# nyenyu12/BioInformatics-project-for-Shotgun-Metagenomics-Pseudo-alignment-shotgun-

Measured on AMD Instinct MI355X. Metric: reads/sec pseudo-aligned (k=31, 150bp) at 1/2/4/8 GPUs; % HBM roofline, higher is better.
Workload: dtype u8

## Files before the change

bioinformatics-project-for-shotgun-metagenomics-pseudo-alignment-shotgun-_amd/csrc/pa_align.hip:

```cpp
#include <hip/hip_runtime.h>

#include <algorithm>
#include <cstdio>
#include <cstdlib>
#include <cstring>
#include <type_traits>
#include <vector>

#include "pa_device.h"
#include "pa_internal.h"

using namespace pad;

namespace {

constexpr int kBlock = 256;
constexpr int kWaves = kBlock / 64;
constexpr uint32_t kSegMaxWaves = 16384;
constexpr uint32_t kSegSlackWaves = 8192, kSegSlackChunks = 5;
constexpr uint64_t kSegSlack = 64ull * kSegSlackChunks * kSegSlackWaves;
constexpr uint32_t kLdsGenomeCap = 2048;

enum : uint32_t { F_MRQ = 1, F_MKQ = 2, F_MG = 4 };

struct AlignArgs {
    const void *table;
    uint64_t cap;
    HomeCfg home;
    uint32_t G;
    int k;
    const uint32_t *class_genomes;
    const uint64_t *class_mask;
    const uint32_t *tile_cls;
    const uint64_t *tile_pk;
    uint64_t tile_n;
    const uint64_t *goff;
    const uint64_t *tile_lw;
    const uint64_t *tile_big;
    const void *tile_nb;
    uint64_t nb_base1, nb_split;
    const uint32_t *nbbig_ld;
    uint64_t nbbig_mask;
    int nb_spec;
    const uint32_t *tile_nbbig;
    const uint4 *tile_nbm;
    int mg_nb;
    const uint32_t *gblk;
    const uint64_t *bloom;
    const uint64_t *tile_rcp;
    const uint32_t *mm_bits;
    uint32_t mm_lg;
    const uint32_t *tile_rcnb;
    uint32_t bloom_lg;
    int walk_rounds;
    int tpos_local;
    uint32_t lane_maxpend;
    int lane_noanchor;
    int dbg_mode;
    const uint8_t *seq;
    const uint8_t *qual;
    const uint64_t *off;
    uint64_t n;
    uint64_t base;
    pa::DevParams prm;
    unsigned long long *stats;
    unsigned long long *uniq;
    unsigned long long *amb;
    unsigned long long *first;
    uint32_t *queue;
    unsigned long long *qcount;
// ... 676 lines not shown
                        uint32_t rank = 0;
                        for (uint32_t u = 0; u < nt; u++) {
                            const uint32_t h = ws.touched[u];
                            rank += h < g && ld_agent(&ws.g_tot[h]) == mx;
                        }
                        if (o + rank < end) x.lists[o + rank] = g;
                    }
                }
            }
            __syncthreads();
            exact_restore(ws, nt, n_touched, n_cls);
        }
        if (threadIdx.x == 0 && x.detail == 1) x.len_out[r] = nc;
        __syncthreads();
    }
}


size_t fast_lds_bytes(uint32_t G, int wpl, bool need_q) {
    size_t cnt = G <= kLdsGenomeCap ? (((size_t)((G + 1) & ~1u) * 16 + 15) / 16 * 16) : 0;
    size_t wl = wpl == 1 ? fast_wave_bytes<1>(need_q) : wpl == 2 ? fast_wave_bytes<2>(need_q) : fast_wave_bytes<4>(need_q);
    return cnt + kWaves * wl;
}

const char *env(const char *name) { return std::getenv(name); }
bool env_is(const char *name, char c) { const char *e = env(name); return e && e[0] == c; }
uint64_t env_u64(const char *name, uint64_t unset) { const char *e = env(name); return e ? std::strtoull(e, nullptr, 10) : unset; }
int env_int(const char *name, int unset) { const char *e = env(name); return e ? std::atoi(e) : unset; }
int env_01(const char *name) { const char *e = env(name); return e ? e[0] == '1' : -1; }

struct Switches {
    bool no_qelide = env("PA_NO_QELIDE");
    bool no_lane = env_is("PA_NO_LANE", '1');
    uint64_t lane_grid = env_u64("PA_LANE_GRID", ~0ull);
    uint32_t lane_maxpend = (uint32_t)env_int("PA_LANE_MAXPEND", 96);
    int lane_noanchor = env_01("PA_LANE_NOANCHOR");
    uint64_t na_min = env_u64("PA_NA_MIN", 32768);
    bool na_seg = !env_is("PA_NA_SEG", '0');
    bool na_rcwalk = !env_is("PA_NA_RCWALK", '0');
    bool na_rcnb = !env_is("PA_NA_RCNB", '0');
    bool mm_bits = !env_is("PA_MM_BITS", '0');
    bool no_nbbig = env("PA_NO_NBBIG");
    bool no_nbm = env("PA_NO_NBM");
    bool no_mgnb = env("PA_NO_MGNB");
    int walk_rounds = env_int("PA_WALK_ROUNDS", 1);
    int dbg_mode = env_int("PA_DBG_MODE", 0);
};

using pa::int_c;
using pa::with_int;
using pa::with_nw;

template <class F>
auto with_filters(uint32_t flags, F &&f) {
    const auto with_mg = [&](auto need_q, auto win_q) {
        return (flags & F_MG) ? f(need_q, win_q, std::true_type{}) : f(need_q, win_q, std::false_type{});
    };
    if (flags & F_MKQ) return with_mg(std::true_type{}, std::true_type{});
    if (flags & F_MRQ) return with_mg(std::true_type{}, std::false_type{});
    return with_mg(std::false_type{}, std::false_type{});
}

template <bool WIN_Q, class F>
auto with_shape(int nw, bool nm4, F &&f) {
    return with_int<3, 2, 1>(nw, [&](auto w) {
        if constexpr (!WIN_Q && w() == 1)
// ... 103 lines not shown
        PA_TRY(resident_grid(kern.rc, kBlock, 0, want, grid));
        PA_TRY(launch_timed(prof, PA_PROF_LANE_RC, kern.rc, grid, 0, st, b));
        b.queue_na = a.queue_na2;
        b.queue_na_count = a.queue_na2_count;
    }
    PA_TRY(resident_grid(kern.na, kBlock, 0, want, grid));
    return launch_timed(prof, PA_PROF_LANE_NA, kern.na, grid, 0, st, b);
}

pa_status launch_exact(pa_index *prof, int nw, const ExactArgs &x, unsigned grid, hipStream_t st) {
    KernelTimer kt(prof, st, PA_PROF_EXACT);
    with_nw(nw, [&](auto w) {
        hipLaunchKernelGGL(k_align_exact<w()>, dim3(grid), dim3(kBlock), 0, st, x);
    });
    PA_HIP(hipGetLastError());
    return PA_OK;
}

constexpr unsigned kExactGrid = 512;

AlignArgs make_args(const pa_index *idx, const pa_reads *r, const pa::DevParams &p, uint64_t base, const Switches &sw) {
    AlignArgs a{};
    a.table = idx->table;
    a.cap = idx->cap;
    a.home = idx->home;
    a.G = idx->n_genomes;
    a.k = (int)std::max<int64_t>(idx->k, 0);
    a.class_genomes = idx->class_genomes;
    a.class_mask = idx->class_mask;
    a.tile_cls = idx->tile_cls;
    a.tile_pk = idx->tile_pk;
    a.goff = idx->goff;
    a.tile_lw = idx->tile_cls ? idx->tile_lw : nullptr;
    a.tile_nb = idx->tile_cls ? idx->tile_nb : nullptr;
    a.nb_spec = idx->nb_spec;
    a.nb_split = idx->tile_nb1 ? idx->nb_split : ~0ull;
    a.nb_base1 = idx->tile_nb1 ? (uint64_t)(uintptr_t)idx->tile_nb1 - idx->nb_split * (idx->nb_spec ? 8 : 4) : 0;
    a.nbbig_ld = (const uint32_t *)(a.tile_nb ? a.tile_nb : (const void *)a.tile_lw);
    a.nbbig_mask = 0;
    a.gblk = idx->tile_gblk;
    a.bloom = idx->tile_cls ? idx->bloom : nullptr;
    a.bloom_lg = idx->bloom_lg;
    a.tile_rcp = idx->tile_cls && sw.na_rcwalk ? idx->tile_rcp : nullptr;
    a.mm_bits = idx->tile_cls && sw.mm_bits ? idx->mm_bits : nullptr;
    a.mm_lg = idx->mm_lg;
    a.tile_rcnb = idx->tile_cls && sw.na_rcnb ? idx->tile_rcnb : nullptr;
    a.tile_n = idx->tile_cls ? idx->tile_n : 0;
    a.walk_rounds = sw.walk_rounds;
    a.tpos_local = idx->tpos_local;
    a.lane_maxpend = sw.lane_maxpend;
    a.lane_noanchor = sw.lane_noanchor < 0 ? a.bloom != nullptr : sw.lane_noanchor;
    a.dbg_mode = sw.dbg_mode;
    a.seq = r->seq;
    a.qual = r->qual;
    a.off = r->off;
    a.n = r->n;
    a.base = base;
    a.prm = p;
    return a;
}

struct DetailOut { uint8_t *type; uint32_t *qf, *hr, *len; const uint64_t *list_off; uint32_t *lists; };

pa_status exact_args(pa_index *idx, const pa_reads *r, const AlignArgs &a, const DetailOut *out, ExactArgs &x,
                     unsigned &grid) {
    const uint32_t wcap = std::max<uint32_t>(1, r->max_len);
// ... 469 lines not shown
```

bioinformatics-project-for-shotgun-metagenomics-pseudo-alignment-shotgun-_amd/csrc/pa_index.hip:

```cpp
#include <hip/hip_runtime.h>

#include <algorithm>
#include <cmath>
#include <cstdlib>
#include <cstring>
#include <chrono>
#include <memory>
#include <cstdio>
#include <string>
#include <vector>

#include "pa_device.h"
#include "pa_internal.h"

using namespace pad;

namespace {

constexpr int kBlock = 256;
constexpr int kRun = 16;
#ifndef PA_BATCHED_INSERT
#define PA_BATCHED_INSERT 1
#endif
constexpr bool kBatchedInsert = PA_BATCHED_INSERT != 0;
// ... 1221 lines not shown
            if (maybe) maybe = table_find<1, true>(table, hc.cap, kk, home_of<1>(kk, key_hash(kk), hc), slot, cls, tpos);
        }
        const uint64_t b = __ballot(maybe);
        if (lane == 0) rcp[j] = b;
    }
}

__global__ void k_mm_build(const Slot<1> *__restrict__ table, uint64_t cap, uint32_t *bits, uint32_t lg, int k) {
    const uint64_t stride = (uint64_t)gridDim.x * blockDim.x;
    for (uint64_t i = (uint64_t)blockIdx.x * blockDim.x + threadIdx.x; i < cap; i += stride) {
        const uint64_t key = table[i].key[0];
        if (key == EMPTY) continue;
        const uint32_t h = mm_bit(k == 31 ? key_minimizer_c<31>(key) : key_minimizer(key, k), lg);
        atomicOr(&bits[h >> 5], 1u << (h & 31));
    }
}

__global__ __launch_bounds__(256) void k_tile_walk(const uint32_t *__restrict__ tile_cls, const uint64_t *__restrict__ pk,
                                                   uint64_t n, uint32_t G, uint64_t *__restrict__ lw, uint64_t n_blocks) {
    const uint32_t lane = threadIdx.x & 63;
    const uint64_t nw = (uint64_t)gridDim.x * (blockDim.x >> 6);
    for (uint64_t j = (uint64_t)blockIdx.x * (blockDim.x >> 6) + (threadIdx.x >> 6); j < n_blocks; j += nw) {
        const uint64_t t = 64 * j + lane;
        const uint32_t v = t < n ? tile_cls[t] : NONE;
        const bool ok = v != NONE, rep = ok && (v & PA_TILE_REP);
        const bool spec = ok && !rep && (v & ~PA_TILE_REP) < G;
        const uint64_t a = __ballot(ok && !rep), b = __ballot(rep || spec);
        if (lane < 4) {
            const uint64_t w = lane == 0 ? (64 * j < n ? pk[2 * j] : 0ull)
                             : lane == 1 ? (64 * j + 32 < n ? pk[2 * j + 1] : 0ull)
                             : lane == 2 ? a : b;
            lw[4 * j + lane] = w;
        }
    }
}

template <int NW>
__global__ void k_table_order(Slot<NW> *table, HomeCfg hc) {
    const uint64_t cap = hc.cap;
    uint64_t i = (uint64_t)blockIdx.x * blockDim.x + threadIdx.x;
    const uint64_t stride = (uint64_t)gridDim.x * blockDim.x;
    for (; i < cap; i += stride) {
        if (table[i].key[0] == EMPTY || table[i == 0 ? cap - 1 : i - 1].key[0] != EMPTY) continue;
        auto at = [&](uint64_t t) { return i + t >= cap ? i + t - cap : i + t; };
        auto rel = [&](const Slot<NW> &s) {
            Key<NW> kk;
#pragma unroll
            for (int j = 0; j < NW; j++) kk.w[j] = s.key[j];
            const uint64_t h = home_of<NW>(kk, key_hash(kk), hc);
            return h >= i ? h - i : h + cap - i;
        };
        for (uint64_t t = 1;; t++) {
            const Slot<NW> x = table[at(t)];
            if (x.key[0] == EMPTY) break;
            const uint64_t hx = rel(x);
            uint64_t q = t;
            for (; q > 0; q--) {
                const Slot<NW> y = table[at(q - 1)];
                if (rel(y) <= hx) break;
                table[at(q)] = y;
            }
            if (q != t) table[at(q)] = x;
        }
    }
}

// ... 462 lines not shown
    size_t free_b = 0, total_b = 0;
    if (!(no_nb && no_nb[0] == '1') && pa::dev_mem_info(&free_b, &total_b) == hipSuccess && bytes <= free_b / 4) {
        PA_HIP(pa::dev_malloc(&idx->tile_nb, bytes));
        PA_HIP(hipMemsetAsync(idx->tile_nb, 0, bytes, st));
        pa::Bufs b(st);
        uint64_t *bb = nullptr;
        uint32_t bb_lg = 6;
        if (idx->n_kmers > 0) {
            while (bb_lg < 33 && (1ull << bb_lg) * 4 < idx->n_kmers) bb_lg++;
            size_t fb = 0, tb = 0;
            if (pa::dev_mem_info(&fb, &tb) != hipSuccess) fb = 0;
            while (bb_lg > 6 && (1ull << bb_lg) * 8 > fb / 4) bb_lg--;
            if ((1ull << bb_lg) * 64 >= idx->n_kmers * 8 && b.get(&bb, (1ull << bb_lg) * 8) == hipSuccess) {
                PA_HIP(hipMemsetAsync(bb, 0, (1ull << bb_lg) * 8, st));
                hipLaunchKernelGGL(k_bloom_build2<3>, dim3(grid_for(idx->cap) > 65536 ? 65536 : grid_for(idx->cap)),
                                   dim3(kBlock), 0, st, (const Slot<3> *)idx->table, idx->cap, bb, bb_lg);
            } else {
                bb = nullptr;
            }
        }
        hipLaunchKernelGGL(k_nb_sum3, dim3(grid_for(n) > 65536 ? 65536 : grid_for(n)), dim3(kBlock), 0, st,
                           idx->tile_pk, idx->tile_cls, n, (int)idx->k, (const Slot<3> *)idx->table, idx->home,
                           (uint32_t *)idx->tile_nb, bb, bb_lg);
        PA_HIP(hipGetLastError());
        PA_HIP(b.free(bb));
        idx->nb_spec = 0;
        idx->device_bytes += bytes;
        phase_mark("nb: three-word summaries");
    }
    idx->nb_pending = 0;
    return PA_OK;
}

template <int NW>
pa_status build_tiles_nw(pa_index *idx, hipStream_t st) {
    const uint32_t G = idx->n_genomes;
    const int k = (int)idx->k;
    const int wpt = build_run();
    const uint64_t mask0 = (2 * k - 64 * (NW - 1)) >= 64 ? ~0ull : ((1ull << (2 * k - 64 * (NW - 1))) - 1);
    Slot<NW> *table = (Slot<NW> *)idx->table;
    if (idx->tile_n > 0) {
        size_t free_b = 0, total_b = 0;
        if (pa::dev_mem_info(&free_b, &total_b) != hipSuccess || idx->tile_n * 7 + (2ull << 30) > free_b) idx->tile_n = 0;
    }
    if (idx->tile_n > 0) {
        const uint64_t n = idx->tile_n, nwords = n / 32 + 32;
        PA_HIP(pa::dev_malloc(&idx->tile_cls, n * 4));
        PA_HIP(pa::dev_malloc(&idx->tile_pk, nwords * 8));
        PA_HIP(hipMemsetAsync(idx->tile_cls, 0xFF, n * 4, st));
        hipLaunchKernelGGL(k_tile_pack, dim3(grid_for(nwords) > 65536 ? 65536 : grid_for(nwords)), dim3(kBlock), 0, st,
                           idx->codes, n, idx->tile_pk, nwords);
        {
            std::vector<uint64_t> ts(G + 1, 0);
            for (uint32_t g = 0; g < G; g++) {
                const uint64_t len = idx->h_goff[g + 1] - idx->h_goff[g];
                ts[g + 1] = ts[g] + ((uint64_t)k > len ? 0 : (len - k + 1 + wpt - 1) / wpt);
            }
            pa::Bufs b(st);
            uint64_t *d_ts = nullptr;
            PA_HIP(b.get(&d_ts, (G + 1) * 8));
            PA_HIP(hipMemcpyAsync(d_ts, ts.data(), (G + 1) * 8, hipMemcpyHostToDevice, st));
            if (ts[G] > 0) {
                hipLaunchKernelGGL(k_tile_cls_all<NW>, dim3(grid_for(ts[G])), dim3(kBlock), 0, st, idx->codes, idx->goff,
                                   d_ts, G, k, mask0, table, idx->home, idx->tile_cls, idx->class_genomes,
                                   idx->tpos_local, wpt);
                PA_HIP(hipGetLastError());
// ... 71 lines not shown
                    idx->bloom_lg = lg;
                    idx->device_bytes += (1ull << lg) * 8;
                }
                phase_mark("Bloom");
            }
            {
                const char *nm = std::getenv("PA_NO_MM");
                const uint32_t lg = 25;
                if (NW == 1 && !(nm && nm[0] == '1') && idx->bloom && idx->n_kmers / 9 <= (1ull << lg) / 4 &&
                    pa::dev_malloc(&idx->mm_bits, (1ull << lg) / 8) == hipSuccess) {
                    PA_HIP(hipMemsetAsync(idx->mm_bits, 0, (1ull << lg) / 8, st));
                    hipLaunchKernelGGL(k_mm_build, dim3(grid_for(idx->cap) > 65536 ? 65536 : grid_for(idx->cap)),
                                       dim3(kBlock), 0, st, (const Slot<1> *)table, idx->cap, idx->mm_bits, lg, k);
                    idx->mm_lg = lg;
                    idx->device_bytes += (1ull << lg) / 8;
                } else {
                    idx->mm_bits = nullptr;
                }
                phase_mark("minimizer bitmap");
            }
            {
                const char *nr = std::getenv("PA_NO_RCP");
                const uint64_t n_blocks = n / 64 + 5;
                if (NW == 1 && !(nr && nr[0] == '1') && pa::dev_malloc(&idx->tile_rcp, n_blocks * 8) == hipSuccess) {
                    hipLaunchKernelGGL(k_tile_rcp, dim3((unsigned)std::min<uint64_t>((n_blocks + 3) / 4, 1u << 20)),
                                       dim3(256), 0, st, idx->tile_cls, idx->tile_pk, n, k, (const Slot<1> *)table,
                                       idx->home, idx->bloom, idx->bloom_lg, idx->tile_rcp, n_blocks);
                    idx->device_bytes += n_blocks * 8;
                } else {
                    idx->tile_rcp = nullptr;
                }
                phase_mark("reverse-complement plane");
            }
        }
        PA_HIP(hipGetLastError());
        PA_HIP(hipStreamSynchronize(st));
        idx->device_bytes += n * 4 + nwords * 8;
    }
    return PA_OK;
}

template <int NW>
pa_status lookup_nw(const pa_index *idx, const uint8_t *d_kmers, uint64_t n, int64_t *d_cls, uint32_t *d_size,
                    hipStream_t st) {
    const int k = (int)idx->k;
    const uint64_t mask0 = (2 * k - 64 * (NW - 1)) >= 64 ? ~0ull : ((1ull << (2 * k - 64 * (NW - 1))) - 1);
    hipLaunchKernelGGL(k_lookup<NW>, dim3(grid_for(n)), dim3(kBlock), 0, st, (const Slot<NW> *)idx->table, idx->home,
                       d_kmers, n, k, mask0, idx->n_genomes, idx->class_genomes, d_cls, d_size);
    PA_HIP(hipGetLastError());
    return PA_OK;
}

template <int NW>
void extsim_slots_nw(const pa_index *idx, const uint32_t *d_group, uint32_t n_groups, unsigned long long *total,
                     unsigned long long *uniq, unsigned long long *ccount, hipStream_t st) {
    int use_lds = n_groups <= 4096;
    size_t shm = use_lds ? (size_t)n_groups * 8 : 0;
    unsigned grid = grid_for(idx->cap) > 4096 ? 4096 : grid_for(idx->cap);
    hipLaunchKernelGGL(k_extsim_slots<NW>, dim3(grid), dim3(kBlock), shm, st, (const Slot<NW> *)idx->table, idx->cap,
                       idx->n_genomes, d_group, n_groups, total, uniq, ccount, use_lds);
}

}

namespace pa {

void index_release(pa_index *idx) {
    index_release_coverage(idx);
    pa::dev_free(idx->table);
    pa::dev_free(idx->class_off);
    pa::dev_free(idx->class_size);
    pa::dev_free(idx->class_genomes);
    pa::dev_free(idx->class_mask);
    pa::dev_free(idx->codes);
    pa::dev_free(idx->goff);
    pa::dev_free(idx->fwd_len);
    idx->fwd_len = nullptr;
    pa::dev_free(idx->tile_cls);
    pa::dev_free(idx->tile_pk);
    pa::dev_free(idx->tile_lw);
    idx->tile_lw = nullptr;
    pa::dev_free(idx->tile_big);
    idx->tile_big = nullptr;
    idx->tile_big_mg = -1;
    pa::dev_free(idx->tile_nb);
    idx->tile_nb = nullptr;
    pa::dev_free(idx->tile_nb1);
    idx->tile_nb1 = nullptr;
    idx->nb_split = ~0ull;
    pa::dev_free(idx->tile_rcnb);
    idx->tile_rcnb = nullptr;
    pa::dev_free(idx->tile_nbbig);
    idx->tile_nbbig = nullptr;
    idx->tile_nbbig_mg = -1;
    pa::dev_free(idx->tile_nbm);
    idx->tile_nbm = nullptr;
    idx->tile_nbm_mg = -1;
    pa::dev_free(idx->bloom);
    idx->bloom = nullptr;
    pa::dev_free(idx->tile_rcp);
    idx->tile_rcp = nullptr;
    pa::dev_free(idx->mm_bits);
    idx->mm_bits = nullptr;
    pa::dev_free(idx->tile_gblk);
    idx->tile_gblk = nullptr;
    idx->bloom_lg = 0;
    idx->tile_cls = nullptr;
    idx->tile_pk = nullptr;
    pa::dev_free(idx->ws.ptr);
    pa::dev_free(idx->queue);
    pa::dev_free(idx->queue_hard);
    pa::dev_free(idx->queue_na);
    pa::dev_free(idx->queue_na2);
    pa::dev_free(idx->queue_na_keys);
// ... 9 lines not shown
    pa::dev_free(idx->qmask);
    pa::dev_free(idx->qdrop);
    idx->qmask = nullptr;
    idx->qdrop = nullptr;
    idx->qmask_cap = 0;
    idx->queue_na = nullptr;
    idx->na_count = nullptr;
    pa::dev_free(idx->counters);
    for (auto e : idx->ev_start) hipEventDestroy(e);
    for (auto e : idx->ev_stop) hipEventDestroy(e);
    for (auto &e : idx->kev) {
        hipEventDestroy(e.start);
        hipEventDestroy(e.stop);
    }
    idx->kev.clear();
    idx->table = nullptr;
}

pa_status index_build_rcnb(pa_index *idx, hipStream_t st) {
    if (!idx->rcnb_pending) return PA_OK;
    std::unique_ptr<PhaseTimer> own;
    if (!t_phase) own.reset(new PhaseTimer(st));
    PhaseScope ps(t_phase ? t_phase : own.get());
    Bufs b(st);
    uint64_t *bb = nullptr;
    uint32_t bb_lg = 6;
    PA_TRY(make_nb_bloom(idx, st, b, &bb, &bb_lg));
    return build_rcnb(idx, st, bb, bb_lg);
}

pa_status index_note_reads(pa_index *idx, uint64_t n, hipStream_t st) {
    idx->reads_seen += n;
    if (!idx->nb_pending || !nb_repaid(idx->reads_seen, idx->tile_n, idx->nw)) return PA_OK;
    return build_nb(idx, st);
}

pa_status index_prepare(pa_index *idx, hipStream_t st, uint64_t reads_hint, bool complete) {
    if (!idx->tiles_pending) {
        if (complete && idx->nb_pending &&
            (reads_hint == ~0ull || nb_repaid(idx->reads_seen + reads_hint, idx->tile_n, idx->nw))) {
            std::unique_ptr<PhaseTimer> own;
            if (!t_phase) own.reset(new PhaseTimer(st));
            PhaseScope ps(t_phase ? t_phase : own.get());
            return build_nb(idx, st);
        }
        return PA_OK;
    }
    idx->tiles_pending = 0;
    std::unique_ptr<PhaseTimer> own;
    if (!t_phase) own.reset(new PhaseTimer(st));
    PhaseScope ps(t_phase ? t_phase : own.get());
    const uint64_t bases = idx->h_goff.empty() ? 0 : idx->h_goff.back();
    idx->nb_skip = reads_hint != ~0ull && !nb_repaid(reads_hint, bases, idx->nw);
    pa_status rc = idx->nw == 3   ? build_tiles_nw<3>(idx, st)
                   : idx->nw == 2 ? build_tiles_nw<2>(idx, st)
                                  : build_tiles_nw<1>(idx, st);
    idx->nb_skip = 0;
    if (rc != PA_OK) {
        pa::dev_free(idx->tile_cls); pa::dev_free(idx->tile_pk); pa::dev_free(idx->tile_lw); pa::dev_free(idx->tile_nb);
        pa::dev_free(idx->tile_nb1);
        idx->tile_nb1 = nullptr, idx->nb_split = ~0ull, idx->rcnb_pending = 0;
        pa::dev_free(idx->tile_gblk); pa::dev_free(idx->bloom); pa::dev_free(idx->tile_rcp); pa::dev_free(idx->tile_rcnb);
        pa::dev_free(idx->mm_bits);
        idx->mm_bits = nullptr;
        idx->tile_rcnb = nullptr;
        idx->tile_cls = nullptr, idx->tile_pk = nullptr, idx->tile_lw = nullptr, idx->tile_nb = nullptr;
        idx->tile_gblk = nullptr, idx->bloom = nullptr, idx->bloom_lg = 0, idx->tile_n = 0, idx->tile_rcp = nullptr;
    }
    return rc;
}

pa_status index_build(pa_index *idx, const char *genomes, const uint64_t *goff, uint32_t n, int64_t k,
                      hipStream_t st, bool defer_tiles, uint8_t *dev_codes) {
    PhaseTimer tm(st);
    PhaseScope ps(&tm);
    idx->k = k;
    idx->nw = k > 0 ? key_words(k) : 1;
    idx->n_genomes = n;
    const bool both = idx->both_strands != 0;
    const uint64_t text_off = goff[0], fwd_total = goff[n] - goff[0];
    std::vector<uint64_t> fwd_goff, region_goff;
    if (both) {
        idx->h_fwd_len.resize(n);
        for (uint32_t g = 0; g < n; g++) {
            const uint64_t len = goff[g + 1] - goff[g];
            idx->h_fwd_len[g] = dev_codes ? (len ? (len - 1) / 2 : 0) : len;
        }
        if (!dev_codes) {
            fwd_goff.assign(goff, goff + n + 1);
            for (auto &o : fwd_goff) o -= goff[0];
            region_goff.assign(n + 1, 0);
            for (uint32_t g = 0; g < n; g++) region_goff[g + 1] = region_goff[g] + strand_region(idx->h_fwd_len[g]);
            goff = region_goff.data();
        }
    }
    idx->h_goff.assign(goff, goff + n + 1);
    const uint64_t total = goff[n] - goff[0];
// ... 367 lines not shown
```

bioinformatics-project-for-shotgun-metagenomics-pseudo-alignment-shotgun-_amd/csrc/pa_internal.h:

```cpp
#pragma once

#include <hip/hip_runtime.h>
#include <stdint.h>

#include <map>
#include <memory>
#include <string>
#include <type_traits>
#include <vector>

#include "../../include/pa.h"
#include "pa_home.h"

namespace pa {

void set_error(const std::string &msg);

pa_status hip_failed(hipError_t e, const char *where);
#define PA_STR2(x) #x
#define PA_STR(x) PA_STR2(x)
#define PA_HIP(call)                                                                              \
    do {                                                                                          \
        hipError_t e_ = (call);                                                                   \
        if (e_ != hipSuccess) return ::pa::hip_failed(e_, __FILE__ ":" PA_STR(__LINE__) " (" #call ")"); \
// ... 114 lines not shown

struct pa_index {
    int device = 0;
    int64_t k = 0;
    int nw = 1;
    uint32_t n_genomes = 0;
    void *table = nullptr;
    uint64_t cap = 0;
    pad::HomeCfg home{};
    uint64_t n_kmers = 0;
    uint64_t n_multi = 0;
    uint64_t *class_off = nullptr;
    uint32_t *class_size = nullptr;
    uint32_t *class_genomes = nullptr;
    uint64_t class_entries = 0;
    uint64_t *class_mask = nullptr;
    uint8_t *codes = nullptr;
    uint64_t *goff = nullptr;
    std::vector<uint64_t> h_goff;
    uint64_t total_windows = 0;
    int tpos_local = 0;
    uint64_t distinct_estimate = 0;
    int released = 0;
    int force_large = 0;
    int compact_table = 0;
    int both_strands = 0;
    std::vector<uint64_t> h_fwd_len;
    uint64_t *fwd_len = nullptr;
    uint64_t tile_n = 0;
    int tiles_pending = 0;
    uint32_t *tile_cls = nullptr;
    uint64_t *tile_pk = nullptr;
    uint64_t *tile_lw = nullptr;
    uint64_t *tile_big = nullptr;
    int64_t tile_big_mg = -1;
    void *tile_nb = nullptr;
    int nb_spec = 0;
    void *tile_nb1 = nullptr;
    uint64_t nb_split = ~0ull;
    uint32_t *tile_rcnb = nullptr;
    int rcnb_pending = 0;
    int rcnb_checks = 0;
    uint32_t *tile_nbbig = nullptr;
    int64_t tile_nbbig_mg = -1;
    uint4 *tile_nbm = nullptr;
    int64_t tile_nbm_mg = -1;
    int nb_skip = 0;
    int nb_pending = 0;
    uint64_t reads_seen = 0;
    uint32_t *tile_gblk = nullptr;
    uint64_t *bloom = nullptr;
    uint32_t *mm_bits = nullptr;
    uint32_t mm_lg = 0;
    uint64_t *tile_rcp = nullptr;
    uint32_t bloom_lg = 0;
    uint64_t device_bytes = 0;
    uint32_t *cov_head = nullptr;
    uint32_t *cov_first = nullptr;
    uint64_t cov_pairs = 0;
    uint64_t cov_bytes = 0;
    int cov_ready = 0;
    uint64_t epoch = 0;
    pa::Workspace ws;
    uint32_t *queue = nullptr;
    uint32_t *queue_hard = nullptr;
    uint32_t *queue_na = nullptr;
// ... 222 lines not shown
```

bioinformatics-project-for-shotgun-metagenomics-pseudo-alignment-shotgun-_amd/csrc/pa_lane.h:

```cpp

constexpr uint64_t kPosMask = (1ull << 40) - 1;
template <int NM>
struct LaneShape {
    static constexpr int MAXW = 64 * NM;
    static constexpr int NWD = NM == 2 ? 6 : 9;
    static constexpr int MAXLEN = 32 * NWD - 16;
    static constexpr int NB = NM + 1;
};
constexpr int kLaneMaxW = LaneShape<2>::MAXW;
constexpr int kLaneMaxLen = LaneShape<2>::MAXLEN;
constexpr int kLaneWords = LaneShape<2>::NWD;
#ifndef PA_LANE_MAXMIS
#define PA_LANE_MAXMIS 40
#endif
constexpr uint32_t kLaneMaxMis = PA_LANE_MAXMIS;
#ifndef PA_LANE_PROBES
#define PA_LANE_PROBES 4
#endif
#ifndef PA_LANE_SEEDS
#define PA_LANE_SEEDS 5
#endif
#ifndef PA_SEED_SLOTS
#define PA_SEED_SLOTS 2
#endif
// ... 220 lines not shown
    uint64_t P[NM];
    uint64_t F[NM];
    uint32_t qf;
    uint32_t uoff;
};

__device__ __forceinline__ uint64_t row_bits(const uint64_t *row, uint32_t o) {
    const uint32_t q = o >> 6, r = o & 63;
    const uint64_t hi = row[q] << r;
    return r ? (hi | (row[q + 1] >> (64 - r))) : hi;
}

template <int NW>
__device__ __forceinline__ Key<NW> row_key(const uint64_t *row, uint32_t w, int k) {
    Key<NW> K;
    if constexpr (NW == 1) {
        K.w[0] = row_bits(row, 2 * w) >> (64 - 2 * k);
    } else {
        static_assert(NW == 2 || NW == 3, "lane-path keys: one to three words");
#pragma unroll
        for (int j = 1; j < NW; j++) K.w[j] = row_bits(row, 2 * w + 2 * k - 64 * (NW - j));
        const int hb = 2 * k - 64 * (NW - 1);
        K.w[0] = hb ? row_bits(row, 2 * w) >> (64 - hb) : 0ull;
    }
    return K;
}

__device__ __forceinline__ uint32_t in_read_mask(uint32_t p0, uint32_t shift, uint32_t len) {
    const uint32_t lo = shift > p0 ? shift - p0 : 0u, hi = shift + len > p0 ? shift + len - p0 : 0u;
    return (hi >= 4 ? 0xFFFFFFFFu : ((1u << (8 * hi)) - 1)) & (lo >= 4 ? 0u : (0xFFFFFFFFu << (8 * lo)));
}


template <bool PLANES, int NWD = kLaneWords, int NB = 3>
__device__ __forceinline__ void lane_blocks(const AlignArgs &a, uint64_t A, uint32_t len, uint64_t (&gw)[NWD + 1],
                                            uint64_t (&pa3)[NB], uint64_t (&pb3)[NB]) {
    const uint64_t *lb = a.tile_lw + 4 * (A >> 6);
    const uint32_t r0 = (uint32_t)(A & 63), o = r0 >> 5, last = r0 + len - 1;
#pragma unroll
    for (int i = 0; i <= NWD; i++) {
        const uint32_t w = o + (uint32_t)i;
        gw[i] = 32 * w <= last ? lb[4 * (w >> 1) + (w & 1)] : 0ull;
    }
    if (PLANES) {
#pragma unroll
        for (int i = 0; i < NB; i++) {
            const ulonglong2 p = *(const ulonglong2 *)(lb + 4 * i + 2);
            pa3[i] = p.x;
            pb3[i] = p.y;
        }
    }
}

template <int NWD = kLaneWords>
__device__ __forceinline__ uint32_t lane_count_mismatches(const uint64_t *row, uint32_t len, uint64_t A,
                                                          const uint64_t (&gw)[NWD + 1]) {
    const uint32_t gr = (uint32_t)(2 * A & 63);
    uint32_t n = 0;
    const uint32_t qlast = (len - 1) >> 5, rl = len - 32 * qlast;
    const uint64_t tail = rl >= 32 ? ~0ull : ~0ull << (64 - 2 * rl);
#pragma unroll
    for (int i = 0; i < NWD; i++) {
        if (32 * i >= (int)len) break;
        const uint64_t gwi = gr ? ((gw[i] << gr) | (gw[i + 1] >> (64 - gr))) : gw[i];
        uint64_t d = row[i] ^ gwi;
        if ((uint32_t)i == qlast) d &= tail;
        n += __popcll((d | (d >> 1)) & 0x5555555555555555ull);
    }
    return n;
}
// ... 183 lines not shown
    for (int i = 1; i < NSEED; i++)
        if (at == i) {
            S.anc = stp[i] | ((uint64_t)sw(i) << 40);
            S.acls = scls[i];
        }
    if (S.acls >= a.G) {
        const int64_t e0 = (int64_t)(S.anc & kPosMask) - (int64_t)(S.anc >> 40);
        int64_t e1 = INT64_MIN, e2 = INT64_MIN;
        uint64_t t1 = 0, t2 = 0;
        uint32_t w1 = 0, c1 = 0, w2 = 0, c2 = 0;
#pragma unroll
        for (int i = 0; i < NSEED; i++) {
            const int64_t Ai = (int64_t)stp[i] - sw(i);
            if (stp[i] == ~0ull || Ai == e0 || Ai == e1 || e2 != INT64_MIN) continue;
            if (e1 == INT64_MIN) {
                e1 = Ai;
                t1 = stp[i], w1 = sw(i), c1 = scls[i];
            } else {
                e2 = Ai;
                t2 = stp[i], w2 = sw(i), c2 = scls[i];
            }
        }
        if (e1 != INT64_MIN) {
#ifdef PA_STATS
            atomicAdd(&a.dbg[26], 1ull);
#endif
#ifndef PA_LANE_RANK_WORDS4
#define PA_LANE_RANK_WORDS4 5
#endif
            constexpr int NR = NM == 2 ? PA_LANE_RANK_WORDS : PA_LANE_RANK_WORDS4;
            const uint32_t rlen = len < 32u * NR ? len : 32u * NR;
            const bool f0 = lane_fits(a, len, e0), f1 = lane_fits(a, len, e1), f2 = e2 != INT64_MIN && lane_fits(a, len, e2);
            uint64_t g0[NR + 1], g1[NR + 1], g2[NR + 1], u3[3];
            lane_blocks<false, NR>(a, f0 ? (uint64_t)e0 : 0, rlen, g0, u3, u3);
            lane_blocks<false, NR>(a, f1 ? (uint64_t)e1 : 0, rlen, g1, u3, u3);
            lane_blocks<false, NR>(a, f2 ? (uint64_t)e2 : 0, rlen, g2, u3, u3);
            const uint32_t m0 = f0 ? lane_count_mismatches<NR>(row, rlen, (uint64_t)e0, g0) : ~0u;
            const uint32_t m1 = f1 ? lane_count_mismatches<NR>(row, rlen, (uint64_t)e1, g1) : ~0u;
            const uint32_t m2 = f2 ? lane_count_mismatches<NR>(row, rlen, (uint64_t)e2, g2) : ~0u;
            uint32_t bj = 0, best = m0;
            if (m1 < best) best = m1, bj = 1;
            if (m2 < best) best = m2, bj = 2;
            if (bj == 1) {
                S.anc = t1 | ((uint64_t)w1 << 40), S.acls = c1;
            } else if (bj == 2) {
                S.anc = t2 | ((uint64_t)w2 << 40), S.acls = c2;
            }
        }
    }
    S.kind = LANE_WALK;
}

template <int NM, bool NEED_Q, bool WIN_Q, bool SEEDS = true, int NW = 1>
__device__ __forceinline__ void lane_prep(const AlignArgs &a, uint64_t r, unsigned long long cd, uint64_t *row,
                                          LaneRead<NM> &S) {
    using SH = LaneShape<NM>;
    static_assert(NM == 2 || !WIN_Q, "the window-quality masks cover 128 windows");
    constexpr int NWD = SH::NWD;
    S.kind = LANE_HARD;
    S.hr = S.nspec = S.nincl = 0;
#pragma unroll
    for (int i = 0; i < NM; i++) S.F[i] = 0;
    S.qf = 0;
    S.uoff = 0;
    const int k = a.k;
    const uint32_t flags = a.prm.flags;
    const uint64_t o = a.off[r];
    const uint32_t len = (uint32_t)(a.off[r + 1] - o);
    const uint64_t o0 = o & ~15ull;
// ... 158 lines not shown
    for (int i = 1; i < NSEED; i++)
        if (at == i) {
            S.anc = stp[i] | ((uint64_t)sw(i) << 40);
            S.acls = scls[i];
        }
    if (S.acls >= a.G) {
        const int64_t e0 = (int64_t)(S.anc & kPosMask) - (int64_t)(S.anc >> 40);
        int64_t e1 = INT64_MIN, e2 = INT64_MIN;
        uint64_t t1 = 0, t2 = 0;
        uint32_t w1 = 0, c1 = 0, w2 = 0, c2 = 0;
#pragma unroll
        for (int i = 0; i < NSEED; i++) {
            const int64_t Ai = (int64_t)stp[i] - sw(i);
            if (stp[i] == ~0ull || Ai == e0 || Ai == e1 || e2 != INT64_MIN) continue;
            if (e1 == INT64_MIN) {
                e1 = Ai;
                t1 = stp[i], w1 = sw(i), c1 = scls[i];
            } else {
                e2 = Ai;
                t2 = stp[i], w2 = sw(i), c2 = scls[i];
            }
        }
        if (e1 != INT64_MIN) {
#ifdef PA_STATS
            atomicAdd(&a.dbg[26], 1ull);
#endif
#ifndef PA_LANE_RANK_WORDS4
#define PA_LANE_RANK_WORDS4 5
#endif
            constexpr int NR = NM == 2 ? PA_LANE_RANK_WORDS : PA_LANE_RANK_WORDS4;
            const uint32_t rlen = len < 32u * NR ? len : 32u * NR;
            const bool f0 = lane_fits(a, len, e0), f1 = lane_fits(a, len, e1), f2 = e2 != INT64_MIN && lane_fits(a, len, e2);
            uint64_t g0[NR + 1], g1[NR + 1], g2[NR + 1], u3[3];
            lane_blocks<false, NR>(a, f0 ? (uint64_t)e0 : 0, rlen, g0, u3, u3);
            lane_blocks<false, NR>(a, f1 ? (uint64_t)e1 : 0, rlen, g1, u3, u3);
            lane_blocks<false, NR>(a, f2 ? (uint64_t)e2 : 0, rlen, g2, u3, u3);
            const uint32_t m0 = f0 ? lane_count_mismatches<NR>(row, rlen, (uint64_t)e0, g0) : ~0u;
            const uint32_t m1 = f1 ? lane_count_mismatches<NR>(row, rlen, (uint64_t)e1, g1) : ~0u;
            const uint32_t m2 = f2 ? lane_count_mismatches<NR>(row, rlen, (uint64_t)e2, g2) : ~0u;
            uint32_t bj = 0, best = m0;
            if (m1 < best) best = m1, bj = 1;
            if (m2 < best) best = m2, bj = 2;
            if (bj == 1) {
                S.anc = t1 | ((uint64_t)w1 << 40), S.acls = c1;
            } else if (bj == 2) {
                S.anc = t2 | ((uint64_t)w2 << 40), S.acls = c2;
            }
        }
    }
    S.kind = LANE_WALK;
}

template <int NM>
__device__ __forceinline__ uint64_t lane_any(const uint64_t (&m)[NM]) {
    uint64_t x = 0;
#pragma unroll
    for (int i = 0; i < NM; i++) x |= m[i];
    return x;
}
template <int NM>
__device__ __forceinline__ uint32_t lane_popc(const uint64_t (&m)[NM]) {
    uint32_t x = 0;
#pragma unroll
    for (int i = 0; i < NM; i++) x += (uint32_t)__popcll(m[i]);
    return x;
}

template <int NM>
__device__ __forceinline__ void range_mask(int32_t lo, int32_t hi, uint64_t (&r)[NM]) {
#pragma unroll
    for (int i = 0; i < NM; i++) {
        const int32_t b = 64 * i, l = lo - b, h = hi - b;
        r[i] = (h < 0 || l > 63) ? 0ull
                                 : ((l <= 0 ? ~0ull : (~0ull << l)) & (h >= 63 ? ~0ull : ((2ull << h) - 1)));
    }
}

template <int NM>
__device__ __forceinline__ void or_at(uint64_t (&m)[NM], uint64_t v, int32_t sft) {
#pragma unroll
    for (int i = 0; i < NM; i++) {
        const int32_t s = sft - 64 * i;
        m[i] |= (s >= 64 || s <= -32) ? 0ull : (s >= 0 ? v << s : v >> (-s));
    }
}

template <int NM>
__device__ __forceinline__ void shifted_planes(const uint64_t (&p)[NM + 1], uint32_t fr, uint64_t (&out)[NM]) {
#pragma unroll
    for (int i = 0; i < NM; i++) out[i] = fr ? (p[i] >> fr) | (p[i + 1] << (64 - fr)) : p[i];
}

template <bool WIN_Q, bool MG, int NW = 1, int SURE = lane_sure(WIN_Q, MG, 2, NW)>
__device__ __forceinline__ void lane_walk_150(const AlignArgs &a, const uint64_t *row, LaneRead<2> &S) {
    const int k = a.k;
    uint32_t W = S.W, len = S.len;
    asm volatile("" : "+v"(W), "+v"(len));
    const uint64_t atp = S.anc & kPosMask;
    const int64_t A = (int64_t)atp - (int64_t)(S.anc >> 40);
    const bool in_tile = A >= 0 && (uint64_t)A + W <= a.tile_n;
    const uint64_t Ac = in_tile ? (uint64_t)A : 0;
    const uint32_t gr = (uint32_t)(2 * Ac & 63);
    uint64_t gw[kLaneWords + 1], pa3[3], pb3[3];
    lane_blocks<true>(a, Ac, len, gw, pa3, pb3);
    const uint32_t g = S.acls < a.G ? S.acls : genome_of(a.goff, a.gblk, atp);
    S.g = g;
    const uint64_t gs = a.goff[g], ge = a.goff[g + 1];
    if (!in_tile || A < (int64_t)gs || (uint64_t)A + W - 1 + k > ge) {
        S.kind = LANE_HARD;
        return (void)LANE_HARD_WHY(4);
    }
    const uint32_t fr = (uint32_t)(Ac & 63);
    const uint64_t PA0 = fr ? (pa3[0] >> fr) | (pa3[1] << (64 - fr)) : pa3[0];
    const uint64_t PA1 = fr ? (pa3[1] >> fr) | (pa3[2] << (64 - fr)) : pa3[1];
    const uint64_t PB0 = fr ? (pb3[0] >> fr) | (pb3[1] << (64 - fr)) : pb3[0];
    const uint64_t PB1 = fr ? (pb3[1] >> fr) | (pb3[2] << (64 - fr)) : pb3[1];
    const uint64_t IX0 = PA0 | PB0, IX1 = PA1 | PB1;
    uint64_t U0 = 0, U1 = 0, V0 = 0, V1 = 0, NP0 = 0, NP1 = 0, NS0 = 0, NS1 = 0, NG0 = 0, NG1 = 0;
    uint32_t nmis = 0;
    const bool has_nb = a.tile_nb != nullptr;
    uint64_t epk = 0;
    uint32_t cpk = 0;
    uint32_t nnb = 0;
    const uint32_t qlast = (len - 1) >> 5, rl = len - 32 * qlast;
    const uint64_t tail = rl >= 32 ? ~0ull : ~0ull << (64 - 2 * rl);
    auto mismatch = [&](uint32_t e, auto &&sub) -> bool {
        const int32_t lo = (int32_t)e - k + 1 < 0 ? 0 : (int32_t)e - k + 1;
        const int32_t hi = (int32_t)e < (int32_t)W - 1 ? (int32_t)e : (int32_t)W - 1;
        if (lo > hi) return true;
        const uint64_t r0 = lo < 64 ? ((~0ull << lo) & (hi >= 63 ? ~0ull : ((2ull << hi) - 1))) : 0ull;
        const uint64_t r1 =
            hi >= 64 ? ((lo <= 64 ? ~0ull : (~0ull << (lo - 64))) & (hi >= 127 ? ~0ull : ((2ull << (hi - 64)) - 1)))
                     : 0ull;
        if (!((r0 & IX0) | (r1 & IX1))) return true;
        if (++nmis > 8) {
            if (nmis > kLaneMaxMis) return false;
            V0 |= r0;
// ... 235 lines not shown
    }
    if ((uint32_t)(__popcll(P0) + __popcll(P1)) > a.lane_maxpend) {
        S.kind = LANE_HARD;
        return (void)LANE_HARD_WHY(8);
    }
}

#ifndef PA_LANE_HALVES
#define PA_LANE_HALVES 1
#endif
template <bool MG>
__device__ __forceinline__ void lane_walk_halves(const AlignArgs &a, const uint64_t *row, LaneRead<4> &S) {
    const int64_t A = (int64_t)(S.anc & kPosMask) - (int64_t)(S.anc >> 40);
    const uint32_t len = S.len, W = S.W;
    S.nspec = S.nincl = S.hr = S.uoff = 0;
    S.P[2] = S.P[3] = 0;
    uint32_t cs = 0, sw = 0;
#pragma unroll 1
    for (uint32_t h = 0; h < 2; h++) {
        LaneRead<2> H;
        H.kind = LANE_WALK;
        H.F[0] = H.F[1] = 0;
        if (h == 0) {
            H.len = W > 128 ? 127 + (uint32_t)a.k : len;
            H.W = W > 128 ? 128u : W;
            H.anc = S.anc;
            H.acls = S.acls;
        } else {
            H.len = len - 128;
            H.W = W - 128;
            H.anc = (uint64_t)(A + 128);
            H.acls = S.g;
        }
        lane_walk_150<false, MG, 1, lane_sure(false, MG, 4, 1) ? 2 : 0>(a, row + 4 * h, H);
        if (h == 0) S.g = H.g;
        S.kind = H.kind;
        S.nspec += H.nspec, S.nincl += H.nincl, S.hr += H.hr, S.uoff += H.uoff & 255u;
        if (H.kind == LANE_WALK && (H.uoff & 0xFF00u)) {
            if (!cs) sw = 128 * h + ((H.uoff >> 16) & 255u);
            cs += (H.uoff >> 8) & 255u;
        }
        if (h == 0) {
            S.P[0] = H.P[0], S.P[1] = H.P[1];
        } else {
            S.P[2] = H.P[0], S.P[3] = H.P[1];
        }
        if (S.kind != LANE_WALK || W <= 128) break;
    }
    if (S.kind == LANE_WALK && cs && S.nspec < cs + (uint32_t)(a.prm.m > 0 ? a.prm.m : 1)) {
#pragma unroll
        for (uint32_t q = 0; q < 4; q++) S.P[q] = (sw >> 6) == q ? 1ull << (sw & 63) : 0ull;
        S.uoff = kLaneSure;
    }
}

template <int NM, bool WIN_Q, bool MG>
__device__ __forceinline__ void lane_walk_long(const AlignArgs &a, const uint64_t *row, LaneRead<NM> &S) {
    using SH = LaneShape<NM>;
    constexpr int NWD = SH::NWD;
    const int k = a.k;
    const uint32_t W = S.W, len = S.len;
    const uint64_t atp = S.anc & kPosMask;
    const int64_t A = (int64_t)atp - (int64_t)(S.anc >> 40);
    const bool in_tile = A >= 0 && (uint64_t)A + W <= a.tile_n;
    const uint64_t Ac = in_tile ? (uint64_t)A : 0;
    const uint32_t gr = (uint32_t)(2 * Ac & 63);
    uint64_t gw[NWD + 1], pa3[NM + 1], pb3[NM + 1];
// ... 1353 lines not shown
```

Baseline: 4.553 billion.

## Add overlapping walk-block records so lane walks read contiguous 128-byte spans

Builds a new device array in which each 64-base tile block gets a 128-byte record holding the packed words and masks of that block and the next three blocks. The lane walk and verification paths index this record instead of gathering up to three separate 32-byte tile_lw entries, so each read's genome window comes from one contiguous span. The cost is a table four times the size of tile_lw, an extra build kernel, and a free-memory check that skips the table when memory is short. It is on by default and can be turned off with PA_LW_RECORDS=0.

Result: no change. 4.554 billion, median of 3 (+0.0%).

```diff
diff --git a/bioinformatics-project-for-shotgun-metagenomics-pseudo-alignment-shotgun-_amd/csrc/pa_align.hip b/bioinformatics-project-for-shotgun-metagenomics-pseudo-alignment-shotgun-_amd/csrc/pa_align.hip
--- a/bioinformatics-project-for-shotgun-metagenomics-pseudo-alignment-shotgun-_amd/csrc/pa_align.hip
+++ b/bioinformatics-project-for-shotgun-metagenomics-pseudo-alignment-shotgun-_amd/csrc/pa_align.hip
@@ -36,6 +36,8 @@
     uint64_t tile_n;
     const uint64_t *goff;
     const uint64_t *tile_lw;
+    const uint64_t *lw_walk;
+    uint32_t lw_sh;
     const uint64_t *tile_big;
     const void *tile_nb;
     uint64_t nb_base1, nb_split;
@@ -778,6 +780,7 @@
 struct Switches {
     bool no_qelide = env("PA_NO_QELIDE");
     bool no_lane = env_is("PA_NO_LANE", '1');
+    bool lw_records = !env_is("PA_LW_RECORDS", '0');
     uint64_t lane_grid = env_u64("PA_LANE_GRID", ~0ull);
     uint32_t lane_maxpend = (uint32_t)env_int("PA_LANE_MAXPEND", 96);
     int lane_noanchor = env_01("PA_LANE_NOANCHOR");
@@ -947,6 +950,9 @@
     a.tile_pk = idx->tile_pk;
     a.goff = idx->goff;
     a.tile_lw = idx->tile_cls ? idx->tile_lw : nullptr;
+    const bool lw_rec = a.tile_lw && idx->tile_lwr && sw.lw_records;
+    a.lw_walk = lw_rec ? idx->tile_lwr : a.tile_lw;
+    a.lw_sh = lw_rec ? 4 : 2;
     a.tile_nb = idx->tile_cls ? idx->tile_nb : nullptr;
     a.nb_spec = idx->nb_spec;
     a.nb_split = idx->tile_nb1 ? idx->nb_split : ~0ull;
diff --git a/bioinformatics-project-for-shotgun-metagenomics-pseudo-alignment-shotgun-_amd/csrc/pa_index.hip b/bioinformatics-project-for-shotgun-metagenomics-pseudo-alignment-shotgun-_amd/csrc/pa_index.hip
--- a/bioinformatics-project-for-shotgun-metagenomics-pseudo-alignment-shotgun-_amd/csrc/pa_index.hip
+++ b/bioinformatics-project-for-shotgun-metagenomics-pseudo-alignment-shotgun-_amd/csrc/pa_index.hip
@@ -1277,6 +1277,17 @@
                              : lane == 2 ? a : b;
             lw[4 * j + lane] = w;
         }
+    }
+}
+
+__global__ __launch_bounds__(256) void k_tile_walk_rec(const uint64_t *__restrict__ lw, uint64_t n_blocks,
+                                                       uint64_t *__restrict__ rec) {
+    const uint64_t stride = (uint64_t)gridDim.x * blockDim.x;
+    for (uint64_t t = (uint64_t)blockIdx.x * blockDim.x + threadIdx.x; t < 8 * n_blocks; t += stride) {
+        const uint64_t b = (t >> 3) + ((t >> 1) & 3);
+        ulonglong2 v = make_ulonglong2(0ull, 0ull);
+        if (b < n_blocks) v = *(const ulonglong2 *)(lw + 4 * b + 2 * (t & 1));
+        *(ulonglong2 *)(rec + 2 * t) = v;
     }
 }
 
@@ -1805,6 +1816,28 @@
     return PA_OK;
 }
 
+pa_status build_lw_records(pa_index *idx, hipStream_t st) {
+    if (!idx->tile_lw || idx->tile_lwr || idx->nb_pending || idx->tile_n == 0) return PA_OK;
+    const char *off = std::getenv("PA_LW_RECORDS"), *mb = std::getenv("PA_LW_RECORDS_MB");
+    if (off && off[0] == '0') return PA_OK;
+    const uint64_t n_blocks = idx->tile_n / 64 + 8, bytes = n_blocks * 128;
+    if (bytes > (mb ? (uint64_t)std::strtoull(mb, nullptr, 10) : 1024ull) << 20) return PA_OK;
+    const uint64_t later = idx->rcnb_pending ? idx->tile_n * 16 : 0;
+    size_t free_b = 0, total_b = 0;
+    if (!(pa::dev_mem_info(&free_b, &total_b) == hipSuccess && bytes + later + (8ull << 30) < free_b &&
+          pa::dev_malloc_try((void **)&idx->tile_lwr, bytes) == hipSuccess)) {
+        (void)hipGetLastError();
+        idx->tile_lwr = nullptr;
+        return PA_OK;
+    }
+    hipLaunchKernelGGL(k_tile_walk_rec, dim3((unsigned)std::min<uint64_t>((8 * n_blocks + 255) / 256, 1u << 20)), dim3(256),
+                       0, st, idx->tile_lw, n_blocks, idx->tile_lwr);
+    PA_HIP(hipGetLastError());
+    idx->device_bytes += bytes;
+    phase_mark("walk-block records");
+    return PA_OK;
+}
+
 template <int NW>
 pa_status build_tiles_nw(pa_index *idx, hipStream_t st) {
     const uint32_t G = idx->n_genomes;
@@ -1942,6 +1975,7 @@
                 }
                 phase_mark("reverse-complement plane");
             }
+            PA_TRY(build_lw_records(idx, st));
         }
         PA_HIP(hipGetLastError());
         PA_HIP(hipStreamSynchronize(st));
@@ -1990,6 +2024,8 @@
     pa::dev_free(idx->tile_pk);
     pa::dev_free(idx->tile_lw);
     idx->tile_lw = nullptr;
+    pa::dev_free(idx->tile_lwr);
+    idx->tile_lwr = nullptr;
     pa::dev_free(idx->tile_big);
     idx->tile_big = nullptr;
     idx->tile_big_mg = -1;
@@ -2065,7 +2101,8 @@
 pa_status index_note_reads(pa_index *idx, uint64_t n, hipStream_t st) {
     idx->reads_seen += n;
     if (!idx->nb_pending || !nb_repaid(idx->reads_seen, idx->tile_n, idx->nw)) return PA_OK;
-    return build_nb(idx, st);
+    PA_TRY(build_nb(idx, st));
+    return build_lw_records(idx, st);
 }
 
 pa_status index_prepare(pa_index *idx, hipStream_t st, uint64_t reads_hint, bool complete) {
@@ -2075,7 +2112,8 @@
             std::unique_ptr<PhaseTimer> own;
             if (!t_phase) own.reset(new PhaseTimer(st));
             PhaseScope ps(t_phase ? t_phase : own.get());
-            return build_nb(idx, st);
+            PA_TRY(build_nb(idx, st));
+            return build_lw_records(idx, st);
         }
         return PA_OK;
     }
@@ -2096,6 +2134,8 @@
         pa::dev_free(idx->tile_gblk); pa::dev_free(idx->bloom); pa::dev_free(idx->tile_rcp); pa::dev_free(idx->tile_rcnb);
         pa::dev_free(idx->mm_bits);
         idx->mm_bits = nullptr;
+        pa::dev_free(idx->tile_lwr);
+        idx->tile_lwr = nullptr;
         idx->tile_rcnb = nullptr;
         idx->tile_cls = nullptr, idx->tile_pk = nullptr, idx->tile_lw = nullptr, idx->tile_nb = nullptr;
         idx->tile_gblk = nullptr, idx->bloom = nullptr, idx->bloom_lg = 0, idx->tile_n = 0, idx->tile_rcp = nullptr;
diff --git a/bioinformatics-project-for-shotgun-metagenomics-pseudo-alignment-shotgun-_amd/csrc/pa_internal.h b/bioinformatics-project-for-shotgun-metagenomics-pseudo-alignment-shotgun-_amd/csrc/pa_internal.h
--- a/bioinformatics-project-for-shotgun-metagenomics-pseudo-alignment-shotgun-_amd/csrc/pa_internal.h
+++ b/bioinformatics-project-for-shotgun-metagenomics-pseudo-alignment-shotgun-_amd/csrc/pa_internal.h
@@ -170,6 +170,7 @@
     uint32_t *tile_cls = nullptr;
     uint64_t *tile_pk = nullptr;
     uint64_t *tile_lw = nullptr;
+    uint64_t *tile_lwr = nullptr;
     uint64_t *tile_big = nullptr;
     int64_t tile_big_mg = -1;
     void *tile_nb = nullptr;
diff --git a/bioinformatics-project-for-shotgun-metagenomics-pseudo-alignment-shotgun-_amd/csrc/pa_lane.h b/bioinformatics-project-for-shotgun-metagenomics-pseudo-alignment-shotgun-_amd/csrc/pa_lane.h
--- a/bioinformatics-project-for-shotgun-metagenomics-pseudo-alignment-shotgun-_amd/csrc/pa_lane.h
+++ b/bioinformatics-project-for-shotgun-metagenomics-pseudo-alignment-shotgun-_amd/csrc/pa_lane.h
@@ -276,10 +276,11 @@
 }
 
 
-template <bool PLANES, int NWD = kLaneWords, int NB = 3>
+template <bool PLANES, int NWD = kLaneWords, int NB = 3, bool REC = true>
 __device__ __forceinline__ void lane_blocks(const AlignArgs &a, uint64_t A, uint32_t len, uint64_t (&gw)[NWD + 1],
                                             uint64_t (&pa3)[NB], uint64_t (&pb3)[NB]) {
-    const uint64_t *lb = a.tile_lw + 4 * (A >> 6);
+    constexpr bool IN4 = REC && (NWD + 1) / 2 <= 3 && (!PLANES || NB <= 4);
+    const uint64_t *lb = IN4 ? a.lw_walk + ((A >> 6) << a.lw_sh) : a.tile_lw + 4 * (A >> 6);
     const uint32_t r0 = (uint32_t)(A & 63), o = r0 >> 5, last = r0 + len - 1;
 #pragma unroll
     for (int i = 0; i <= NWD; i++) {
@@ -529,9 +530,9 @@
             const uint32_t rlen = len < 32u * NR ? len : 32u * NR;
             const bool f0 = lane_fits(a, len, e0), f1 = lane_fits(a, len, e1), f2 = e2 != INT64_MIN && lane_fits(a, len, e2);
             uint64_t g0[NR + 1], g1[NR + 1], g2[NR + 1], u3[3];
-            lane_blocks<false, NR>(a, f0 ? (uint64_t)e0 : 0, rlen, g0, u3, u3);
-            lane_blocks<false, NR>(a, f1 ? (uint64_t)e1 : 0, rlen, g1, u3, u3);
-            lane_blocks<false, NR>(a, f2 ? (uint64_t)e2 : 0, rlen, g2, u3, u3);
+            lane_blocks<false, NR, 3, NM == 2>(a, f0 ? (uint64_t)e0 : 0, rlen, g0, u3, u3);
+            lane_blocks<false, NR, 3, NM == 2>(a, f1 ? (uint64_t)e1 : 0, rlen, g1, u3, u3);
+            lane_blocks<false, NR, 3, NM == 2>(a, f2 ? (uint64_t)e2 : 0, rlen, g2, u3, u3);
             const uint32_t m0 = f0 ? lane_count_mismatches<NR>(row, rlen, (uint64_t)e0, g0) : ~0u;
             const uint32_t m1 = f1 ? lane_count_mismatches<NR>(row, rlen, (uint64_t)e1, g1) : ~0u;
             const uint32_t m2 = f2 ? lane_count_mismatches<NR>(row, rlen, (uint64_t)e2, g2) : ~0u;
@@ -756,9 +757,9 @@
             const uint32_t rlen = len < 32u * NR ? len : 32u * NR;
             const bool f0 = lane_fits(a, len, e0), f1 = lane_fits(a, len, e1), f2 = e2 != INT64_MIN && lane_fits(a, len, e2);
             uint64_t g0[NR + 1], g1[NR + 1], g2[NR + 1], u3[3];
-            lane_blocks<false, NR>(a, f0 ? (uint64_t)e0 : 0, rlen, g0, u3, u3);
-            lane_blocks<false, NR>(a, f1 ? (uint64_t)e1 : 0, rlen, g1, u3, u3);
-            lane_blocks<false, NR>(a, f2 ? (uint64_t)e2 : 0, rlen, g2, u3, u3);
+            lane_blocks<false, NR, 3, NM == 2>(a, f0 ? (uint64_t)e0 : 0, rlen, g0, u3, u3);
+            lane_blocks<false, NR, 3, NM == 2>(a, f1 ? (uint64_t)e1 : 0, rlen, g1, u3, u3);
+            lane_blocks<false, NR, 3, NM == 2>(a, f2 ? (uint64_t)e2 : 0, rlen, g2, u3, u3);
             const uint32_t m0 = f0 ? lane_count_mismatches<NR>(row, rlen, (uint64_t)e0, g0) : ~0u;
             const uint32_t m1 = f1 ? lane_count_mismatches<NR>(row, rlen, (uint64_t)e1, g1) : ~0u;
             const uint32_t m2 = f2 ? lane_count_mismatches<NR>(row, rlen, (uint64_t)e2, g2) : ~0u;
@@ -815,7 +816,7 @@
     for (int i = 0; i < NM; i++) out[i] = fr ? (p[i] >> fr) | (p[i + 1] << (64 - fr)) : p[i];
 }
 
-template <bool WIN_Q, bool MG, int NW = 1, int SURE = lane_sure(WIN_Q, MG, 2, NW)>
+template <bool WIN_Q, bool MG, int NW = 1, int SURE = lane_sure(WIN_Q, MG, 2, NW), bool REC = true>
 __device__ __forceinline__ void lane_walk_150(const AlignArgs &a, const uint64_t *row, LaneRead<2> &S) {
     const int k = a.k;
     uint32_t W = S.W, len = S.len;
@@ -826,7 +827,7 @@
     const uint64_t Ac = in_tile ? (uint64_t)A : 0;
     const uint32_t gr = (uint32_t)(2 * Ac & 63);
     uint64_t gw[kLaneWords + 1], pa3[3], pb3[3];
-    lane_blocks<true>(a, Ac, len, gw, pa3, pb3);
+    lane_blocks<true, kLaneWords, 3, REC>(a, Ac, len, gw, pa3, pb3);
     const uint32_t g = S.acls < a.G ? S.acls : genome_of(a.goff, a.gblk, atp);
     S.g = g;
     const uint64_t gs = a.goff[g], ge = a.goff[g + 1];
@@ -1128,7 +1129,7 @@
             H.anc = (uint64_t)(A + 128);
             H.acls = S.g;
         }
-        lane_walk_150<false, MG, 1, lane_sure(false, MG, 4, 1) ? 2 : 0>(a, row + 4 * h, H);
+        lane_walk_150<false, MG, 1, lane_sure(false, MG, 4, 1) ? 2 : 0, false>(a, row + 4 * h, H);
         if (h == 0) S.g = H.g;
         S.kind = H.kind;
         S.nspec += H.nspec, S.nincl += H.nincl, S.hr += H.hr, S.uoff += H.uoff & 255u;
```
